# eduardburlacu/DiTSep

Hardware: AMD Instinct MI355X
Metric: separated utterances/sec @ N=30, 2-spk 4 s mixtures (higher is better)
Workload: dtype fp16 (fp16 MFMA operands, fp32 accumulate)

## Files before the change

ditsep_amd/csrc/common.h:

```cpp
#pragma once
#include <hip/hip_runtime.h>
#include <stdint.h>

typedef unsigned short op16_t;
typedef __attribute__((ext_vector_type(8))) unsigned short op16x8;
typedef __attribute__((ext_vector_type(4))) unsigned short op16x4;
typedef __attribute__((ext_vector_type(8))) __bf16 bf16x8;
typedef __attribute__((ext_vector_type(8))) _Float16 f16x8;
typedef __attribute__((ext_vector_type(4))) float f32x4;

#define DSN_WAVE 64

#define DSN_PL(planes, f16) ((planes) | ((f16) << 4))
#define PL_COUNT(pl) ((pl)&3)
#define PL_F16(pl) ((pl) >> 4)

enum { DSN_ACT_NONE = 0, DSN_ACT_ELU = 1, DSN_ACT_SNAKE = 2, DSN_ACT_SILU = 3 };
enum { DSN_F32_NONE = 0, DSN_F32_TANH = 1 };

__device__ __forceinline__ float dsn_elu(float v) { return v > 0.f ? v : expm1f(v); }
__device__ __forceinline__ float dsn_silu(float v) { return v / (1.f + __expf(-v)); }
__device__ __forceinline__ float dsn_snake(float v, float alpha, float inv_beta) {
  float s = __sinf(v * alpha);
  return v + inv_beta * s * s;
}

#define DSN_F16_MAX 65504.f
__device__ __forceinline__ float dsn_sat16(float v) {
  const float c = __builtin_amdgcn_fmed3f(v, -DSN_F16_MAX, DSN_F16_MAX);
  return v != v ? v : c;
}
__device__ __forceinline__ op16_t to_op16(float v, int f16) {
  return f16 ? __builtin_bit_cast(unsigned short, (_Float16)dsn_sat16(v)) : __builtin_bit_cast(unsigned short, (__bf16)v);
}
__device__ __forceinline__ float from_op16(op16_t u, int f16) {
// ... 167 lines not shown
```

ditsep_amd/csrc/engine.hip:

```cpp
#include <math.h>
#include <stdarg.h>
#include <stdio.h>
#include <stdlib.h>
#include <string.h>

#include <algorithm>
#include <map>
#include <numeric>
#include <set>
#include <stdexcept>
#include <string>
#include <vector>

#include "../../include/ditsep_hip.h"
#include "dit_plan.h"
#include "igemm.h"
#include "kernels.h"
#include "resample_plan.h"
#include "score_window.h"

namespace {

struct Err : std::runtime_error {
  int code;
// ... 4241 lines not shown
                 (int)h[i], (long)h[i] * t->mul, t->L);
        const char* why = launch_codec_tail_zero(oplanes, t->out_ps, P, t->x, t->out_f32, t->B, t->L, t->C,
                                                 reinterpret_cast<const int*>(t->lens), t->rep, t->mul, st);
        if (why) fail(DSN_EINVAL, "test_kernel codec_tail_zero: %s (C=%d)", why, t->C);
        break;
      }
      case DSN_TK_RANDN:
      case DSN_TK_RAND_UNIFORM: {
        const char* nm = t->kind == DSN_TK_RANDN ? "randn" : "rand_uniform";
        if (t->count < 1) fail(DSN_EINVAL, "test_kernel %s: count %ld must be positive", nm, (long)t->count);
        if (!t->out_f32) fail(DSN_EINVAL, "test_kernel %s: out_f32 missing", nm);
        if (t->kind == DSN_TK_RANDN) launch_randn(t->out_f32, (long)t->count, t->seed, t->offset, st);
        else launch_rand_uniform(t->out_f32, (long)t->count, t->seed, t->offset, t->lo, t->hi, st);
        break;
      }
      case DSN_TK_WN_SCALE: {
        if (t->rows < 1 || t->count < 1)
          fail(DSN_EINVAL, "test_kernel wn_scale: rows and count must be positive (rows=%d count=%ld)", t->rows, (long)t->count);
        if (!t->x || !t->gamma || !t->out_f32) fail(DSN_EINVAL, "test_kernel wn_scale: x (v), gamma (g) or out_f32 missing");
        launch_wn_scale(t->x, t->gamma, t->out_f32, t->rows, (long)t->count, st);
        break;
      }
      case DSN_TK_PACK_WEIGHT: {
        static const char* const modes[] = {"linear", "linear_swiglu", "conv", "convt", "conv2d", "nin"};
        const int m = t->mode, N = t->N, K = t->K;
        if (m < PACK_LINEAR || m > PACK_NIN) fail(DSN_EINVAL, "test_kernel pack_weight: unknown mode %d", m);
        if (N < 1 || K < 1) fail(DSN_EINVAL, "test_kernel pack_weight %s: N and K must be positive (N=%d K=%d)", modes[m], N, K);
        if (!t->x || !oplanes) fail(DSN_EINVAL, "test_kernel pack_weight %s: x (the source) or out_planes missing", modes[m]);
        if (t->out_ps < (long)N * K) fail(DSN_EINVAL, "test_kernel pack_weight %s: out_ps %ld < N*K", modes[m], (long)t->out_ps);
        const bool linear = m == PACK_LINEAR || m == PACK_LINEAR_SWIGLU;
// ... 279 lines not shown
```

ditsep_amd/csrc/kernels.h:

```cpp
#pragma once
#include "common.h"

void launch_pack_tokens(const float* src0, int C0, const float* src1, int C1, int B, int T,
                        float* dst_f32, op16_t* dst_planes, long ps, int planes, hipStream_t s);
void launch_win_pack_tokens(const float* src0, int C0, const float* src1, int C1, const int* wtab, int W, int Tw,
                            int Tsrc, float* dst_f32, op16_t* dst_planes, long ps, int planes, hipStream_t s);
void launch_win_times(const float* t, const int* wtab, int W, float* tw, hipStream_t s);
void launch_win_blend_tokens(const float* src, const int* ftab, const float* fw, float* out, long rows, int C, int Tw,
                             hipStream_t s);
void launch_copy_rows(const float* src, float* dst, int rows, int width, long dst_stride, hipStream_t s);
void launch_unpack_tokens(const float* src, float* dst, int B, int C, int T, hipStream_t s);
void launch_to_planes(const float* src, op16_t* dst, long ps, int planes, long n, hipStream_t s);

void launch_pc_prior(const float* mean, int mean_full, const float* z, float* x, float stdT, int B, int n, int D,
                     int T, hipStream_t s);
void launch_pc_corrector(float* x, float* x_mean , const float* score_tok, const float* z, float step,
                         float noise_gain, const float* norms, float snr, int B, int n, int D, int T, hipStream_t s);
void launch_pc_item_norms(const float* a, long per_item, int B, float* out, hipStream_t s);
void launch_pc_predictor(float* x, float* x_mean, const float* y, const float* score_tok, const float* z,
                         float theta, float dt, float G, float g, int em, int B, int n, int D, int T, hipStream_t s);

void launch_sigma_mix(const float* y, float* smix, int B, int L, int avg_len, hipStream_t s);
void launch_mix_prior(const float* y, const float* z, float* x, const float* smix, float s1, float s2, int B, int n, int D,
                      int T, hipStream_t s);
// ... 10 lines not shown
void launch_residual_norm(float* x, const float* slabs, int nslab, long slab_stride, const float* bias,
                          const float* gamma, const float* beta, op16_t* out, long ps, int planes, int rows, int D,
                          float eps, int do_norm, hipStream_t s, unsigned char* out_fp8_scale = nullptr);
void launch_timestep_features(const float* t, const float* w, int B, int half, op16_t* out, long ps,
                              int planes, hipStream_t s);
hipError_t launch_attention_mfma(const op16_t* qkv, long ps, op16_t* out, long out_ps, int pl, int B, int S, int H,
                                 int dh, hipStream_t s, unsigned char* out_fp8_scale = nullptr,
                                 const int* lens = nullptr);
void launch_rope_tables(float* cos_t, float* sin_t, int S, int rot, hipStream_t s);

void launch_conv_out1(const op16_t* a, long ps, int planes, const float* w, float* out, int S, int L, int C,
                      int ktaps, int apply_tanh, hipStream_t s);
void launch_conv_in1(const float* wav, const float* w, const float* bias, int S, int L, int Cout, int ktaps,
                     float* out_f32, op16_t* out_planes, long ps, int planes, int act, const float* act_a,
                     const float* act_b, hipStream_t s);
void launch_vae_sample(const float* enc_tok, const float* noise, float* y, int S, int D, int T, hipStream_t s);

const char* launch_codec_tail_zero(op16_t* planes, long ps, int n_planes, float* xf, float* out, int S, int L, int C,
                                   const int* frames, int rep, int mul, hipStream_t s);
void launch_vae_sample_ragged(const float* enc_tok, const float* noise, const int* frames, float* y, int S, int D, int T,
                              hipStream_t s);

void launch_randn(float* out, long n, unsigned long long seed, unsigned long long offset, hipStream_t s);

enum { PACK_LINEAR = 0, PACK_LINEAR_SWIGLU = 1, PACK_CONV = 2, PACK_CONVT = 3, PACK_CONV2D = 4, PACK_NIN = 5 };
void launch_wn_scale(const float* v, const float* g, float* scale, int R, long inner, hipStream_t s);
void launch_pack_weight(const float* src, const float* scale, op16_t* dst, long ps, int planes, int mode,
                        int N, int K, int Cin, int Cout, int kw, int stride, hipStream_t s,
                        const float* colscale = nullptr);
void launch_packed_row_sum(const op16_t* w, long ps, int planes, int N, int K, float* out, hipStream_t s);
// ... 246 lines not shown
```

ditsep_amd/csrc/kernels.hip:

```cpp
#include "kernels.h"

namespace {

constexpr int TPB = 256;
inline int grid_for(long n, int per_block = TPB, int cap = 256 * 16) {
  long g = (n + per_block - 1) / per_block;
  return (int)(g < 1 ? 1 : (g > cap ? cap : g));
}


template <bool WIN>
__global__ void pack_tokens_kernel(const float* __restrict__ s0, int C0, const float* __restrict__ s1, int C1,
                                   int B, int T, float* __restrict__ df, op16_t* __restrict__ dp, long ps,
                                   int planes, const int* __restrict__ wtab, int Tsrc) {
  const int C = C0 + C1;
  const long n = (long)B * T * C;
  for (long i = blockIdx.x * (long)blockDim.x + threadIdx.x; i < n; i += (long)gridDim.x * blockDim.x) {
    const int c = (int)(i % C);
    const long bt = i / C;
    const int t = (int)(bt % T);
    const int b = (int)(bt / T);
    float v;
    if (WIN) {
      const int r = wtab[3 * b], ts = wtab[3 * b + 1] + t;
// ... 606 lines not shown
      if (q == 0) part[r * 8 + t] = x;
    }
  }
  __syncthreads();
  for (int p = threadIdx.x; p < TILE; p += blockDim.x) {
    const int l = l0 + p;
    if (l < L) {
      float v = 0.f;
#pragma unroll
      for (int t = 0; t < KT; ++t) v += part[(p + t) * 8 + t];
      out[(long)s * L + l] = apply_tanh ? tanhf(v) : v;
    }
  }
}

__global__ void conv_in1_kernel(const float* __restrict__ wav, const float* __restrict__ w,
                                const float* __restrict__ bias, int L, int Cout, int ktaps,
                                float* __restrict__ of, op16_t* __restrict__ op, long ps, int planes, int act,
                                const float* __restrict__ aa, const float* __restrict__ ab, long total) {
  const int pad = (ktaps - 1) / 2;
  for (long i = blockIdx.x * (long)blockDim.x + threadIdx.x; i < total; i += (long)gridDim.x * blockDim.x) {
    const int co = (int)(i % Cout);
    const long sl = i / Cout;
    const int l = (int)(sl % L);
    const long s = sl / L;
    float acc = bias ? bias[co] : 0.f;
    for (int t = 0; t < ktaps; ++t) {
      const int li = l + t - pad;
      if (li >= 0 && li < L) acc += w[co * ktaps + t] * wav[s * L + li];
    }
    if (of) of[i] = acc;
    if (op) {
      float a = acc;
      if (act == DSN_ACT_ELU) a = dsn_elu(acc);
      else if (act == DSN_ACT_SNAKE) a = dsn_snake(acc, aa[co], ab[co]);
      dsn_store_planes1(op, ps, planes, i, a);
    }
  }
}

__global__ void conv_in1_vec_kernel(const float* __restrict__ wav, const float* __restrict__ w,
                                    const float* __restrict__ bias, int L, int Cout, int ktaps,
                                    float* __restrict__ of, op16_t* __restrict__ op, long ps, int planes, int act,
                                    const float* __restrict__ aa, const float* __restrict__ ab, long rows) {
  const int cq = Cout >> 2;
  const int c4 = (threadIdx.x % cq) * 4;
  const int pad = (ktaps - 1) / 2;
  float wr[4][8];
  f32x4 bv = {0.f, 0.f, 0.f, 0.f};
#pragma unroll
  for (int r = 0; r < 4; ++r) {
#pragma unroll
    for (int t = 0; t < 8; ++t) wr[r][t] = t < ktaps ? w[(c4 + r) * ktaps + t] : 0.f;
    if (bias) bv[r] = bias[c4 + r];
  }
  const int rpb = blockDim.x / cq;
  for (long row = blockIdx.x * (long)rpb + threadIdx.x / cq; row < rows; row += (long)gridDim.x * rpb) {
    const int l = (int)(row % L);
    const long s = row / L;
// ... 3 lines not shown
      const int li = l + t - pad;
      x[t] = (t < ktaps && li >= 0 && li < L) ? wav[s * L + li] : 0.f;
    }
    f32x4 acc = bv;
#pragma unroll
    for (int r = 0; r < 4; ++r)
#pragma unroll
      for (int t = 0; t < 8; ++t) acc[r] += wr[r][t] * x[t];
    const long o = row * Cout + c4;
    if (of) *reinterpret_cast<f32x4*>(of + o) = acc;
    if (op) {
      op16x4 hi, lo;
#pragma unroll
      for (int r = 0; r < 4; ++r) {
        float v = acc[r];
        if (act == DSN_ACT_ELU) v = dsn_elu(v);
        else if (act == DSN_ACT_SNAKE) v = dsn_snake(v, aa[c4 + r], ab[c4 + r]);
        op16_t h, lw;
        dsn_split(v, h, lw, PL_F16(planes));
        hi[r] = h;
        lo[r] = lw;
      }
      *reinterpret_cast<op16x4*>(op + o) = hi;
      if (PL_COUNT(planes) == 2) *reinterpret_cast<op16x4*>(op + ps + o) = lo;
    }
  }
}

__global__ void vae_sample_kernel(const float* __restrict__ enc, const float* __restrict__ noise,
                                  float* __restrict__ y, int D, int T, long total) {
  for (long i = blockIdx.x * (long)blockDim.x + threadIdx.x; i < total; i += (long)gridDim.x * blockDim.x) {
    const int t = (int)(i % T);
    const long sc = i / T;
    const int c = (int)(sc % D);
    const long s = sc / D;
    const float* row = enc + (s * T + t) * (2L * D);
    const float mean = row[c], scale = row[D + c];
    const float sp = scale > 20.f ? scale : log1pf(expf(scale));
    y[i] = noise[i] * (sp + 1e-4f) + mean;
  }
// ... 342 lines not shown
                     apply_tanh);
}
void launch_conv_in1(const float* wav, const float* w, const float* bias, int S, int L, int Cout, int ktaps,
                     float* of, op16_t* op, long ps, int planes, int act, const float* aa, const float* ab,
                     hipStream_t st) {
  if (Cout % 4 == 0 && TPB % (Cout / 4) == 0 && ktaps <= 8) {
    const long rows = (long)S * L;
    hipLaunchKernelGGL(conv_in1_vec_kernel, dim3(grid_for(rows * (Cout / 4))), dim3(TPB), 0, st, wav, w, bias, L, Cout,
                       ktaps, of, op, ps, planes, act, aa, ab, rows);
    return;
  }
  const long total = (long)S * L * Cout;
  hipLaunchKernelGGL(conv_in1_kernel, dim3(grid_for(total)), dim3(TPB), 0, st, wav, w, bias, L, Cout, ktaps, of, op,
                     ps, planes, act, aa, ab, total);
}
void launch_vae_sample(const float* enc, const float* noise, float* y, int S, int D, int T, hipStream_t st) {
  const long total = (long)S * D * T;
  hipLaunchKernelGGL(vae_sample_kernel, dim3(grid_for(total)), dim3(TPB), 0, st, enc, noise, y, D, T, total);
}
void launch_randn(float* out, long n, unsigned long long seed, unsigned long long offset, hipStream_t st) {
  hipLaunchKernelGGL(randn_kernel, dim3(grid_for((n + 3) / 4)), dim3(TPB), 0, st, out, n, seed, offset);
}
void launch_rand_uniform(float* out, long n, unsigned long long seed, unsigned long long offset, float lo, float hi,
                         hipStream_t st) {
  hipLaunchKernelGGL(rand_uniform_kernel, dim3(grid_for(n)), dim3(TPB), 0, st, out, n, seed, offset, lo, hi);
}
void launch_wn_scale(const float* v, const float* g, float* scale, int R, long inner, hipStream_t st) {
  hipLaunchKernelGGL(wn_scale_kernel, dim3(cdiv(R, 4)), dim3(TPB), 0, st, v, g, scale, R, inner);
}
void launch_pack_weight(const float* src, const float* scale, op16_t* dst, long ps, int planes, int mode, int N,
// ... 71 lines not shown
```

ditsep_amd/csrc/ru_fused.hip:

```cpp
#include "igemm.h"
#include "kernels.h"
#include <cstdlib>
#include <functional>

namespace {

constexpr int C = 128;
constexpr int TL = 128;
constexpr int KT = 32;
constexpr int WTILE = 128 * KT;
constexpr int NSTW = 3;

__device__ __forceinline__ int swz32(int row, int chunk) { return chunk ^ ((-(row >> 2)) & 3); }

template <int P, int F16>
__global__ __launch_bounds__(256, 2) void ru_fused_kernel(const RuDesc d, const op16_t* __restrict__ zero_page) {
  extern __shared__ __attribute__((aligned(16))) op16_t lds[];
  const int halo = 3 * d.dil;
  const int hrows = (TL + 2 * halo + 3) & ~3;
  constexpr int AH_ROWS = TL + 54 + 2;
  constexpr int AH_PLANE = AH_ROWS * C;
  op16_t* ah = lds;
  op16_t* ring = lds + P * AH_PLANE;
  constexpr int RING_STAGE = P * WTILE;

  const int tid = threadIdx.x, lane = tid & 63;
  const int wave = __builtin_amdgcn_readfirstlane(tid >> 6);
  const int wm = wave >> 1, wn = wave & 1;
  const int tiles_per_seq = (d.L + TL - 1) / TL;
  const int s = blockIdx.x / tiles_per_seq;
// ... 73 lines not shown
#pragma unroll
      for (int tm = 0; tm < 4; ++tm) {
        if (P == 2) {
          acc[tn][tm] = mfma16<F16>(fw[P - 1][tn], fa[0][tm], acc[tn][tm]);
          acc[tn][tm] = mfma16<F16>(fw[0][tn], fa[P - 1][tm], acc[tn][tm]);
        }
        acc[tn][tm] = mfma16<F16>(fw[0][tn], fa[0][tm], acc[tn][tm]);
      }
  }
  asm volatile("s_waitcnt lgkmcnt(0)" ::: "memory");
  __builtin_amdgcn_s_barrier();

  issue_w(d.W1, d.w1_ps, C, 0, 0);
  issue_w(d.W1, d.w1_ps, C, KT, 1);
  const int nq = (lane >> 4) * 4;
#pragma unroll
  for (int tm = 0; tm < 4; ++tm) {
    const int m = wm * 64 + tm * 16 + (lane & 15);
#pragma unroll
    for (int tn = 0; tn < 4; ++tn) {
      const int n = wn * 64 + tn * 16 + nq;
      f32x4 v = acc[tn][tm] + *reinterpret_cast<const f32x4*>(d.b7 + n);
      op16x4 hi, lo;
#pragma unroll
      for (int r = 0; r < 4; ++r) {
        float a = v[r];
        if (d.act_mid == DSN_ACT_ELU) a = dsn_elu(a);
        else if (d.act_mid == DSN_ACT_SNAKE) a = dsn_snake(a, d.mid_a[n + r], d.mid_b[n + r]);
        op16_t h, l;
        dsn_split(a, h, l, F16);
        hi[r] = h;
        lo[r] = l;
      }
      const int off = m * C + (((n >> 3) + 2 * m) & 15) * 8 + (n & 7);
      *reinterpret_cast<op16x4*>(ah + off) = hi;
      if (P == 2) *reinterpret_cast<op16x4*>(ah + AH_PLANE + off) = lo;
      acc[tn][tm] = f32x4{0.f, 0.f, 0.f, 0.f};
    }
  }

  constexpr int NKT1 = C / KT;
  for (int i = 0; i < NKT1; ++i) {
    if (i + 1 < NKT1)
      asm volatile("s_waitcnt vmcnt(%0) lgkmcnt(0)" ::"n"(G) : "memory");
    else
      asm volatile("s_waitcnt vmcnt(0) lgkmcnt(0)" ::: "memory");
    __builtin_amdgcn_s_barrier();
    if (i + 2 < NKT1) issue_w(d.W1, d.w1_ps, C, (i + 2) * KT, (i + 2) % NSTW);
// ... 7 lines not shown
        fa[p][k] = *reinterpret_cast<const op16x8*>(ah + p * AH_PLANE + row * C + ((i * 4 + fchunk + 2 * row) & 15) * 8);
        fw[p][k] = *reinterpret_cast<const op16x8*>(wb + p * WTILE + w_frag + k * 16 * KT);
      }
#pragma unroll
    for (int tn = 0; tn < 4; ++tn)
#pragma unroll
      for (int tm = 0; tm < 4; ++tm) {
        if (P == 2) {
          acc[tn][tm] = mfma16<F16>(fw[P - 1][tn], fa[0][tm], acc[tn][tm]);
          acc[tn][tm] = mfma16<F16>(fw[0][tn], fa[P - 1][tm], acc[tn][tm]);
        }
        acc[tn][tm] = mfma16<F16>(fw[0][tn], fa[0][tm], acc[tn][tm]);
      }
  }

  f32x4 res[4], nres[4];
  auto load_res = [&](int tm, f32x4 (&r)[4]) {
    const int l = l0 + wm * 64 + tm * 16 + (lane & 15);
    const long rowoff = seq_off + (long)min(l, d.L - 1) * C;
#pragma unroll
    for (int tn = 0; tn < 4; ++tn) r[tn] = *reinterpret_cast<const f32x4*>(d.X + rowoff + wn * 64 + tn * 16 + nq);
  };
  load_res(0, res);
#pragma unroll
  for (int tm = 0; tm < 4; ++tm) {
    if (tm + 1 < 4) load_res(tm + 1, nres);
    const int l = l0 + wm * 64 + tm * 16 + (lane & 15);
    const long rowoff = seq_off + (long)l * C;
#pragma unroll
    for (int tn = 0; tn < 4; ++tn) {
      if (l >= d.L) continue;
      const int n = wn * 64 + tn * 16 + nq;
      f32x4 v = acc[tn][tm] + *reinterpret_cast<const f32x4*>(d.b1 + n) + res[tn];
      if (d.out_f32) *reinterpret_cast<f32x4*>(d.out_f32 + rowoff + n) = v;
      if (d.out_planes) {
        op16x4 hi, lo;
#pragma unroll
        for (int r = 0; r < 4; ++r) {
          float a = v[r];
          if (d.act_out == DSN_ACT_ELU) a = dsn_elu(a);
          else if (d.act_out == DSN_ACT_SNAKE) a = dsn_snake(a, d.out_a[n + r], d.out_b[n + r]);
          op16_t h, lw;
          dsn_split(a, h, lw, F16);
          hi[r] = h;
          lo[r] = lw;
        }
        *reinterpret_cast<op16x4*>(d.out_planes + rowoff + n) = hi;
        if (P == 2) *reinterpret_cast<op16x4*>(d.out_planes + d.out_ps + rowoff + n) = lo;
      }
    }
#pragma unroll
    for (int tn = 0; tn < 4; ++tn) res[tn] = nres[tn];
  }
}

constexpr int TL2 = 256;
constexpr int ACH_ROWS = 384;
constexpr int ACH_STAGE = ACH_ROWS * KT;
constexpr int RING2_OFF = 2 * ACH_STAGE;
constexpr int H_ELEMS = TL2 * C;
constexpr int LDS2_ELEMS = H_ELEMS + 2 * WTILE;

template <int F16>
__global__ __launch_bounds__(512, 4) void ru_fused2_kernel(const RuDesc d, const op16_t* __restrict__ zero_page) {
  extern __shared__ __attribute__((aligned(16))) op16_t lds[];
  const int halo = 3 * d.dil;
  const int tid = threadIdx.x, lane = tid & 63;
  const int wave = __builtin_amdgcn_readfirstlane(tid >> 6);
  const int wm = wave >> 1, wn = wave & 1;
  const int tiles_per_seq = (d.L + TL2 - 1) / TL2;
  const int s = blockIdx.x / tiles_per_seq;
  const int l0 = (blockIdx.x - s * tiles_per_seq) * TL2;
  const long seq_off = (long)s * d.L * C;
  const int nrows = TL2 + 2 * halo;

  const op16_t* a_src[3];
#pragma unroll
  for (int j = 0; j < 3; ++j) {
// ... 63 lines not shown
      }
#pragma unroll
      for (int tn = 0; tn < 4; ++tn)
#pragma unroll
        for (int tm = 0; tm < 4; ++tm) acc[tn][tm] = mfma16<F16>(fw[tn], fa[tm], acc[tn][tm]);
      if (++st == NSTW) st = 0;
    }
  }
  asm volatile("s_waitcnt lgkmcnt(0)" ::: "memory");
  __builtin_amdgcn_s_barrier();

  op16_t* ring1 = lds + H_ELEMS;
  issue_w(d.W1, C, 0, ring1);
  issue_w(d.W1, C, KT, ring1 + WTILE);
  const int nq = (lane >> 4) * 4;
#pragma unroll
  for (int tm = 0; tm < 4; ++tm) {
    const int m = wm * 64 + tm * 16 + (lane & 15);
#pragma unroll
    for (int tn = 0; tn < 4; ++tn) {
      const int n = wn * 64 + tn * 16 + nq;
      f32x4 v = acc[tn][tm] + *reinterpret_cast<const f32x4*>(d.b7 + n);
      op16x4 hi;
#pragma unroll
      for (int r = 0; r < 4; ++r) {
        float a = v[r];
        if (d.act_mid == DSN_ACT_ELU) a = dsn_elu(a);
        else if (d.act_mid == DSN_ACT_SNAKE) a = dsn_snake(a, d.mid_a[n + r], d.mid_b[n + r]);
        op16_t h, l;
        dsn_split(a, h, l, F16);
        hi[r] = h;
      }
      *reinterpret_cast<op16x4*>(lds + m * C + (((n >> 3) + 2 * m) & 15) * 8 + (n & 7)) = hi;
      const int ls = l0 + wm * 64 + tm * 16 + (lane & 15);
      acc[tn][tm] = *reinterpret_cast<const f32x4*>(d.b1 + n) +
                    *reinterpret_cast<const f32x4*>(d.X + seq_off + (long)min(ls, d.L - 1) * C + n);
    }
  }

#pragma unroll
  for (int i = 0; i < 4; ++i) {
    if (i == 0)
      asm volatile("s_waitcnt vmcnt(1) lgkmcnt(0)" ::: "memory");
    else
      asm volatile("s_waitcnt vmcnt(0) lgkmcnt(0)" ::: "memory");
    __builtin_amdgcn_s_barrier();
    if (i >= 1 && i + 1 < 4) issue_w(d.W1, C, (i + 1) * KT, ring1 + ((i + 1) & 1) * WTILE);
    const op16_t* wb = ring1 + (i & 1) * WTILE;
    op16x8 fa[4], fw[4];
#pragma unroll
    for (int k = 0; k < 4; ++k) {
      const int row = wm * 64 + k * 16 + frow;
      fa[k] = *reinterpret_cast<const op16x8*>(lds + row * C + ((i * 4 + fchunk + 2 * row) & 15) * 8);
      fw[k] = *reinterpret_cast<const op16x8*>(wb + w_frag + k * 16 * KT);
    }
#pragma unroll
    for (int tn = 0; tn < 4; ++tn)
#pragma unroll
      for (int tm = 0; tm < 4; ++tm) acc[tn][tm] = mfma16<F16>(fw[tn], fa[tm], acc[tn][tm]);
  }

#pragma unroll
  for (int tm = 0; tm < 4; ++tm) {
    const int l = l0 + wm * 64 + tm * 16 + (lane & 15);
    const long rowoff = seq_off + (long)l * C;
#pragma unroll
    for (int tn = 0; tn < 4; ++tn) {
      if (l >= d.L) continue;
      const int n = wn * 64 + tn * 16 + nq;
      const f32x4 v = acc[tn][tm];
      if (d.out_f32) *reinterpret_cast<f32x4*>(d.out_f32 + rowoff + n) = v;
      if (d.out_planes) {
        op16x4 hi;
#pragma unroll
        for (int r = 0; r < 4; ++r) {
          float a = v[r];
          if (d.act_out == DSN_ACT_ELU) a = dsn_elu(a);
          else if (d.act_out == DSN_ACT_SNAKE) a = dsn_snake(a, d.out_a[n + r], d.out_b[n + r]);
          op16_t h, lw;
          dsn_split(a, h, lw, F16);
          hi[r] = h;
        }
        *reinterpret_cast<op16x4*>(d.out_planes + rowoff + n) = hi;
      }
    }
  }
}

template <int P, int F16>
hipError_t launch_t(const RuDesc& d, hipStream_t st) {
  const op16_t* zp = dsn_zero_page();
  if (!zp) return hipErrorOutOfMemory;
  const size_t smem = ((size_t)P * (TL + 56) * C + (size_t)NSTW * P * WTILE) * sizeof(op16_t);
  dsn_allow_lds<ru_fused_kernel<P, F16>>();
  const int grid = d.S * ((d.L + TL - 1) / TL);
  hipLaunchKernelGGL((ru_fused_kernel<P, F16>), dim3(grid), dim3(256), smem, st, d, zp);
  return hipGetLastError();
}

}

template <int F16>
hipError_t launch2_t(const RuDesc& d, hipStream_t st) {
  const op16_t* zp = dsn_zero_page();
  if (!zp) return hipErrorOutOfMemory;
  const size_t smem = (size_t)LDS2_ELEMS * sizeof(op16_t);
  dsn_allow_lds<ru_fused2_kernel<F16>>();
  const int grid = d.S * ((d.L + TL2 - 1) / TL2);
  hipLaunchKernelGGL((ru_fused2_kernel<F16>), dim3(grid), dim3(512), smem, st, d, zp);
  return hipGetLastError();
}

static bool ru_act_ok(int kind, const float* a, const float* b) {
  if (kind == DSN_ACT_SNAKE) return a && b;
  return kind == DSN_ACT_NONE || kind == DSN_ACT_ELU;
}

hipError_t ru_fused_launch(const RuDesc& d, int pl, bool v1, hipStream_t st) {
  if (d.dil < 1 || d.dil > 9 || d.S <= 0 || d.L <= 0) return hipErrorInvalidValue;
  if (!d.A || !d.X || !d.W7 || !d.W1 || !d.b7 || !d.b1 || (!d.out_f32 && !d.out_planes)) return hipErrorInvalidValue;
  if (!ru_act_ok(d.act_mid, d.mid_a, d.mid_b)) return hipErrorInvalidValue;
  if (d.out_planes && !ru_act_ok(d.act_out, d.out_a, d.out_b)) return hipErrorInvalidValue;
  const int P = PL_COUNT(pl), f16 = PL_F16(pl);
  if (d.out_planes) {
    const long n = (long)d.S * d.L * C;
    for (int p = 0; p < P; ++p)
      for (int q = 0; q < P; ++q) {
        const op16_t *a = d.A + p * d.a_ps, *o = d.out_planes + q * d.out_ps;
        if (std::less<const op16_t*>()(a, o + n) && std::less<const op16_t*>()(o, a + n)) return hipErrorInvalidValue;
      }
  }
  if (P == 1 && !v1) return f16 ? launch2_t<1>(d, st) : launch2_t<0>(d, st);
  if (P == 1) return f16 ? launch_t<1, 1>(d, st) : launch_t<1, 0>(d, st);
  return f16 ? launch_t<2, 1>(d, st) : launch_t<2, 0>(d, st);
}
```

ditsep_amd/native.py:

```python
from __future__ import annotations

import ctypes as C
import math
import os
import warnings
from typing import Mapping, Optional

import torch

_HERE = os.path.dirname(os.path.abspath(__file__))
LIB_PATH = os.environ.get("DSN_LIB", os.path.join(_HERE, "libditsep_hip.so"))

PREC_BF16 = 1
PREC_BF16X3 = 2
PREC_FP16 = 3
PREC_FP16X3 = 4
PREC_FP8 = 5
SCORE_NONE, SCORE_DIT, SCORE_NCSNPP = 0, 1, 2
MAX_VAE_BLOCKS = 8

EXPORTS = [
    "dsn_create", "dsn_destroy", "dsn_last_error", "dsn_load_tensor", "dsn_finalize_weights", "dsn_finalize_weights_ex",
    "dsn_score", "dsn_score_ragged", "dsn_pc_sample_ragged", "dsn_decode_ragged", "dsn_encode_ragged",
    "dsn_separate_ragged", "dsn_ouve_schedule", "dsn_pc_sample", "dsn_pc_sample_sched", "dsn_pc_sample_ex", "dsn_pc_sample_mix", "dsn_sb_sample", "dsn_decode",
# ... 134 lines not shown
        ("sc_Cin", C.c_int), ("sc_row_elems", C.c_int),
        ("out_f32", C.c_void_p), ("out_planes", C.c_void_p), ("out_ps", C.c_int64),
        ("slabs", C.c_void_p), ("slab_stride", C.c_int64),
    ]


TEST_KERNEL_KINDS = {"attention": 1, "qkv_attention": 2, "residual_norm": 3, "gn_stats": 4, "gn_apply": 5, "fir2d": 6,
                     "conv_out1": 7, "conv_in1": 8, "ru_fused": 9,
                     "pc_prior": 10, "pc_corrector": 11, "pc_item_norms": 12, "pc_predictor": 13, "sigma_mix": 14,
                     "mix_prior": 15, "mix_corrector": 16, "mix_predictor": 17, "sb_update": 18, "repeat_sources": 19,
                     "vae_sample": 20, "randn": 21, "rand_uniform": 22, "codec_tail_zero": 23,
                     "wn_scale": 24, "pack_weight": 25, "pack_bias_swiglu": 26, "pack_weight_fp8": 27,
                     "packed_row_sum": 28, "fp8_row_sum": 29, "bias_plus_wbeta": 30, "snake_params": 31,
                     "pack_tokens": 32, "unpack_tokens": 33, "copy_rows": 34, "to_planes": 35, "zero_tail": 36,
                     "vae_sample_ragged": 37, "timestep_features": 38, "rope_tables": 39, "ncsn_pack": 40,
                     "ncsn_fourier": 41, "ncsn_output": 42, "win_pack_tokens": 43, "win_blend_tokens": 44}
PACK_MODES = {"linear": 0, "linear_swiglu": 1, "conv": 2, "convt": 3, "conv2d": 4, "nin": 5}


class DsnTestKernel(C.Structure):
    _fields_ = [
        ("kind", C.c_int), ("B", C.c_int), ("S", C.c_int), ("H", C.c_int), ("dh", C.c_int), ("D", C.c_int),
        ("ipp", C.c_int), ("rows", C.c_int), ("nslab", C.c_int), ("do_norm", C.c_int), ("eps", C.c_float),
        ("slab_stride", C.c_int64),
        ("C", C.c_int), ("HW", C.c_int), ("rstride", C.c_int), ("img_h", C.c_int), ("img_w", C.c_int), ("up", C.c_int),
        ("silu", C.c_int), ("bstride", C.c_int64),
        ("L", C.c_int), ("ktaps", C.c_int), ("apply_tanh", C.c_int), ("act", C.c_int),
        ("dil", C.c_int), ("act_out", C.c_int),
        ("a", C.c_void_p), ("a_numel", C.c_int64), ("w", C.c_void_p), ("w_numel", C.c_int64), ("w2", C.c_void_p),
        ("w2_numel", C.c_int64), ("x", C.c_void_p),
        ("slabs", C.c_void_p), ("bias", C.c_void_p), ("bias2", C.c_void_p), ("gamma", C.c_void_p), ("beta", C.c_void_p),
# ... 1880 lines not shown
```

include/ditsep_hip.h:

```cpp
#ifndef DITSEP_HIP_H
#define DITSEP_HIP_H

#include <stdint.h>

#ifdef __cplusplus
extern "C" {
#endif

#define DSN_OK 0
#define DSN_EINVAL (-1)
#define DSN_EHIP (-2)
#define DSN_ESTATE (-3)
#define DSN_ENOMEM (-4)
#define DSN_ESOLVER (-5)

#define DSN_PREC_BF16 1
#define DSN_PREC_BF16X3 2
#define DSN_PREC_FP16 3
#define DSN_PREC_FP16X3 4
#define DSN_PREC_FP8 5

#define DSN_SCORE_NONE 0
#define DSN_SCORE_DIT 1
#define DSN_SCORE_NCSNPP 2
// ... 302 lines not shown
  int64_t slab_stride;
} DsnTestGemm;
int dsn_test_gemm(dsn_ctx* ctx, const DsnTestGemm* t, void* stream);

enum { DSN_TK_ATTENTION = 1, DSN_TK_QKV_ATTENTION = 2, DSN_TK_RESIDUAL_NORM = 3, DSN_TK_GN_STATS = 4,
       DSN_TK_GN_APPLY = 5, DSN_TK_FIR2D = 6, DSN_TK_CONV_OUT1 = 7, DSN_TK_CONV_IN1 = 8, DSN_TK_RU_FUSED = 9,
       DSN_TK_PC_PRIOR = 10, DSN_TK_PC_CORRECTOR = 11, DSN_TK_PC_ITEM_NORMS = 12, DSN_TK_PC_PREDICTOR = 13,
       DSN_TK_SIGMA_MIX = 14, DSN_TK_MIX_PRIOR = 15, DSN_TK_MIX_CORRECTOR = 16, DSN_TK_MIX_PREDICTOR = 17,
       DSN_TK_SB_UPDATE = 18, DSN_TK_REPEAT_SOURCES = 19, DSN_TK_VAE_SAMPLE = 20, DSN_TK_RANDN = 21,
       DSN_TK_RAND_UNIFORM = 22, DSN_TK_CODEC_TAIL_ZERO = 23,
       DSN_TK_WN_SCALE = 24, DSN_TK_PACK_WEIGHT = 25, DSN_TK_PACK_BIAS_SWIGLU = 26, DSN_TK_PACK_WEIGHT_FP8 = 27,
       DSN_TK_PACKED_ROW_SUM = 28, DSN_TK_FP8_ROW_SUM = 29, DSN_TK_BIAS_PLUS_WBETA = 30, DSN_TK_SNAKE_PARAMS = 31,
       DSN_TK_PACK_TOKENS = 32, DSN_TK_UNPACK_TOKENS = 33, DSN_TK_COPY_ROWS = 34, DSN_TK_TO_PLANES = 35,
       DSN_TK_ZERO_TAIL = 36, DSN_TK_VAE_SAMPLE_RAGGED = 37, DSN_TK_TIMESTEP_FEATURES = 38, DSN_TK_ROPE_TABLES = 39,
       DSN_TK_NCSN_PACK = 40, DSN_TK_NCSN_FOURIER = 41, DSN_TK_NCSN_OUTPUT = 42, DSN_TK_WIN_PACK_TOKENS = 43,
       DSN_TK_WIN_BLEND_TOKENS = 44 };
enum { DSN_PACK_LINEAR = 0, DSN_PACK_LINEAR_SWIGLU = 1, DSN_PACK_CONV = 2, DSN_PACK_CONVT = 3, DSN_PACK_CONV2D = 4,
       DSN_PACK_NIN = 5 };
typedef struct DsnTestKernel {
  int kind;
  int B, S, H, dh, D, ipp;
  int rows, nslab, do_norm;
  float eps;
  int64_t slab_stride;
  int C, HW, rstride, img_h, img_w, up, silu;
  int64_t bstride;
  int L, ktaps, apply_tanh, act;
  int dil, act_out;
  const float* a;
  int64_t a_numel;
  const float* w;
// ... 74 lines not shown
```

Before: 290.6.

## Specialize residual-unit epilogues by activation mode and inline a branch-free ELU expm1

Replaces the library expm1f in ELU with an inlined Cody-Waite plus polynomial expm1 for non-positive inputs, adding a sweep kernel that compares it bit-for-bit against the reference. The fused residual-unit kernels and the conv_in1 kernels are templated on activation mode, so the activation and output-pointer branches resolve at compile time. Snake alpha/beta are loaded once as vectors instead of per element. This cuts per-element branching and scalar parameter loads in the epilogues, at the cost of more kernel instantiations and code size.

```diff
diff --git a/ditsep_amd/csrc/common.h b/ditsep_amd/csrc/common.h
--- a/ditsep_amd/csrc/common.h
+++ b/ditsep_amd/csrc/common.h
@@ -18,7 +18,28 @@
 enum { DSN_ACT_NONE = 0, DSN_ACT_ELU = 1, DSN_ACT_SNAKE = 2, DSN_ACT_SILU = 3 };
 enum { DSN_F32_NONE = 0, DSN_F32_TANH = 1 };
 
-__device__ __forceinline__ float dsn_elu(float v) { return v > 0.f ? v : expm1f(v); }
+__device__ __forceinline__ float dsn_expm1_nonpos(float x) {
+  const auto c = [](unsigned bits) { return __builtin_bit_cast(float, bits); };
+  const float t = __builtin_rintf(x * c(0x3fb8aa3bu));
+  float r = __builtin_fmaf(t, c(0xbf317218u), x);
+  r = __builtin_fmaf(t, c(0x3102e308u), r);
+  float p = __builtin_fmaf(c(0x395133b1u), r, c(0x3ab69700u));
+  p = __builtin_fmaf(r, p, c(0x3c0887f9u));
+  p = __builtin_fmaf(r, p, c(0x3d2aaa81u));
+  p = __builtin_fmaf(r, p, c(0x3e2aaaabu));
+  p = __builtin_fmaf(r, p, 0.5f);
+  const float q = r * p;
+  const float u = __builtin_fmaf(r, q, r);
+  const float s = __builtin_amdgcn_ldexpf(1.0f, (int)t);
+  const float y = __builtin_fmaf(s, u, s - 1.0f);
+  return x < -17.0f ? -1.0f : y;
+}
+__device__ __forceinline__ float dsn_elu(float v) {
+  float e = dsn_expm1_nonpos(v > 0.f ? 0.f : v);
+  asm("" : "+v"(e));
+  return v > 0.f ? v : e;
+}
+__device__ __forceinline__ float dsn_elu_ref(float v) { return v > 0.f ? v : expm1f(v); }
 __device__ __forceinline__ float dsn_silu(float v) { return v / (1.f + __expf(-v)); }
 __device__ __forceinline__ float dsn_snake(float v, float alpha, float inv_beta) {
   float s = __sinf(v * alpha);
diff --git a/ditsep_amd/csrc/engine.hip b/ditsep_amd/csrc/engine.hip
--- a/ditsep_amd/csrc/engine.hip
+++ b/ditsep_amd/csrc/engine.hip
@@ -4279,6 +4279,15 @@
         else launch_rand_uniform(t->out_f32, (long)t->count, t->seed, t->offset, t->lo, t->hi, st);
         break;
       }
+      case DSN_TK_ELU_SWEEP: {
+        if (t->count < 1 || t->count > (1ll << 32) || t->offset + (uint64_t)t->count > (1ull << 32))
+          fail(DSN_EINVAL, "test_kernel elu_sweep: patterns offset .. offset + count - 1 must lie in [0, 2^32) (count=%ld)",
+               (long)t->count);
+        if (!t->out_f32 || (reinterpret_cast<uintptr_t>(t->out_f32) & 7))
+          fail(DSN_EINVAL, "test_kernel elu_sweep: out_f32 (16 bytes, 8-byte aligned) missing");
+        launch_elu_sweep(t->offset, (unsigned long long)t->count, reinterpret_cast<unsigned long long*>(t->out_f32), st);
+        break;
+      }
       case DSN_TK_WN_SCALE: {
         if (t->rows < 1 || t->count < 1)
           fail(DSN_EINVAL, "test_kernel wn_scale: rows and count must be positive (rows=%d count=%ld)", t->rows, (long)t->count);
diff --git a/ditsep_amd/csrc/kernels.h b/ditsep_amd/csrc/kernels.h
--- a/ditsep_amd/csrc/kernels.h
+++ b/ditsep_amd/csrc/kernels.h
@@ -48,6 +48,7 @@
 void launch_conv_in1(const float* wav, const float* w, const float* bias, int S, int L, int Cout, int ktaps,
                      float* out_f32, op16_t* out_planes, long ps, int planes, int act, const float* act_a,
                      const float* act_b, hipStream_t s);
+void launch_elu_sweep(unsigned long long first, unsigned long long count, unsigned long long* res, hipStream_t s);
 void launch_vae_sample(const float* enc_tok, const float* noise, float* y, int S, int D, int T, hipStream_t s);
 
 const char* launch_codec_tail_zero(op16_t* planes, long ps, int n_planes, float* xf, float* out, int S, int L, int C,
diff --git a/ditsep_amd/csrc/kernels.hip b/ditsep_amd/csrc/kernels.hip
--- a/ditsep_amd/csrc/kernels.hip
+++ b/ditsep_amd/csrc/kernels.hip
@@ -644,10 +644,11 @@
   }
 }
 
-__global__ void conv_in1_kernel(const float* __restrict__ wav, const float* __restrict__ w,
-                                const float* __restrict__ bias, int L, int Cout, int ktaps,
-                                float* __restrict__ of, op16_t* __restrict__ op, long ps, int planes, int act,
-                                const float* __restrict__ aa, const float* __restrict__ ab, long total) {
+template <int ACT>
+__device__ __forceinline__ void conv_in1_loop(const float* __restrict__ wav, const float* __restrict__ w,
+                                              const float* __restrict__ bias, int L, int Cout, int ktaps,
+                                              float* __restrict__ of, op16_t* __restrict__ op, long ps, int planes,
+                                              const float* __restrict__ aa, const float* __restrict__ ab, long total) {
   const int pad = (ktaps - 1) / 2;
   for (long i = blockIdx.x * (long)blockDim.x + threadIdx.x; i < total; i += (long)gridDim.x * blockDim.x) {
     const int co = (int)(i % Cout);
@@ -662,17 +663,26 @@
     if (of) of[i] = acc;
     if (op) {
       float a = acc;
-      if (act == DSN_ACT_ELU) a = dsn_elu(acc);
-      else if (act == DSN_ACT_SNAKE) a = dsn_snake(acc, aa[co], ab[co]);
+      if (ACT == DSN_ACT_ELU) a = dsn_elu(acc);
+      else if (ACT == DSN_ACT_SNAKE) a = dsn_snake(acc, aa[co], ab[co]);
       dsn_store_planes1(op, ps, planes, i, a);
     }
   }
 }
-
-__global__ void conv_in1_vec_kernel(const float* __restrict__ wav, const float* __restrict__ w,
-                                    const float* __restrict__ bias, int L, int Cout, int ktaps,
-                                    float* __restrict__ of, op16_t* __restrict__ op, long ps, int planes, int act,
-                                    const float* __restrict__ aa, const float* __restrict__ ab, long rows) {
+__global__ void conv_in1_kernel(const float* __restrict__ wav, const float* __restrict__ w,
+                                const float* __restrict__ bias, int L, int Cout, int ktaps,
+                                float* __restrict__ of, op16_t* __restrict__ op, long ps, int planes, int act,
+                                const float* __restrict__ aa, const float* __restrict__ ab, long total) {
+  if (act == DSN_ACT_ELU) conv_in1_loop<DSN_ACT_ELU>(wav, w, bias, L, Cout, ktaps, of, op, ps, planes, aa, ab, total);
+  else if (act == DSN_ACT_SNAKE) conv_in1_loop<DSN_ACT_SNAKE>(wav, w, bias, L, Cout, ktaps, of, op, ps, planes, aa, ab, total);
+  else conv_in1_loop<DSN_ACT_NONE>(wav, w, bias, L, Cout, ktaps, of, op, ps, planes, aa, ab, total);
+}
+
+template <int ACT>
+__device__ __forceinline__ void conv_in1_vec_loop(const float* __restrict__ wav, const float* __restrict__ w,
+                                                  const float* __restrict__ bias, int L, int Cout, int ktaps,
+                                                  float* __restrict__ of, op16_t* __restrict__ op, long ps, int planes,
+                                                  const float* __restrict__ aa, const float* __restrict__ ab, long rows) {
   const int cq = Cout >> 2;
   const int c4 = (threadIdx.x % cq) * 4;
   const int pad = (ktaps - 1) / 2;
@@ -706,8 +716,8 @@
 #pragma unroll
       for (int r = 0; r < 4; ++r) {
         float v = acc[r];
-        if (act == DSN_ACT_ELU) v = dsn_elu(v);
-        else if (act == DSN_ACT_SNAKE) v = dsn_snake(v, aa[c4 + r], ab[c4 + r]);
+        if (ACT == DSN_ACT_ELU) v = dsn_elu(v);
+        else if (ACT == DSN_ACT_SNAKE) v = dsn_snake(v, aa[c4 + r], ab[c4 + r]);
         op16_t h, lw;
         dsn_split(v, h, lw, PL_F16(planes));
         hi[r] = h;
@@ -716,6 +726,33 @@
       *reinterpret_cast<op16x4*>(op + o) = hi;
       if (PL_COUNT(planes) == 2) *reinterpret_cast<op16x4*>(op + ps + o) = lo;
     }
+  }
+}
+__global__ void conv_in1_vec_kernel(const float* __restrict__ wav, const float* __restrict__ w,
+                                    const float* __restrict__ bias, int L, int Cout, int ktaps,
+                                    float* __restrict__ of, op16_t* __restrict__ op, long ps, int planes, int act,
+                                    const float* __restrict__ aa, const float* __restrict__ ab, long rows) {
+  if (act == DSN_ACT_ELU) conv_in1_vec_loop<DSN_ACT_ELU>(wav, w, bias, L, Cout, ktaps, of, op, ps, planes, aa, ab, rows);
+  else if (act == DSN_ACT_SNAKE) conv_in1_vec_loop<DSN_ACT_SNAKE>(wav, w, bias, L, Cout, ktaps, of, op, ps, planes, aa, ab, rows);
+  else conv_in1_vec_loop<DSN_ACT_NONE>(wav, w, bias, L, Cout, ktaps, of, op, ps, planes, aa, ab, rows);
+}
+
+__global__ void elu_sweep_kernel(unsigned long long first, unsigned long long count, unsigned long long* __restrict__ res) {
+  unsigned long long bad = 0, lowest = ~0ull;
+  for (unsigned long long i = blockIdx.x * (unsigned long long)blockDim.x + threadIdx.x; i < count;
+       i += (unsigned long long)gridDim.x * blockDim.x) {
+    const unsigned pat = (unsigned)(first + i);
+    const float v = __builtin_bit_cast(float, pat);
+    const float got = dsn_elu(v), want = dsn_elu_ref(v);
+    const bool same = __builtin_bit_cast(unsigned, got) == __builtin_bit_cast(unsigned, want) || (got != got && want != want);
+    if (!same) {
+      ++bad;
+      lowest = pat < lowest ? pat : lowest;
+    }
+  }
+  if (bad) {
+    atomicAdd(res, bad);
+    atomicMin(res + 1, lowest);
   }
 }
 
@@ -1088,6 +1125,11 @@
   hipLaunchKernelGGL(conv_in1_kernel, dim3(grid_for(total)), dim3(TPB), 0, st, wav, w, bias, L, Cout, ktaps, of, op,
                      ps, planes, act, aa, ab, total);
 }
+void launch_elu_sweep(unsigned long long first, unsigned long long count, unsigned long long* res, hipStream_t st) {
+  (void)hipMemsetAsync(res, 0, sizeof *res, st);
+  (void)hipMemsetAsync(res + 1, 0xff, sizeof *res, st);
+  hipLaunchKernelGGL(elu_sweep_kernel, dim3(grid_for((long)((count + 15) / 16))), dim3(TPB), 0, st, first, count, res);
+}
 void launch_vae_sample(const float* enc, const float* noise, float* y, int S, int D, int T, hipStream_t st) {
   const long total = (long)S * D * T;
   hipLaunchKernelGGL(vae_sample_kernel, dim3(grid_for(total)), dim3(TPB), 0, st, enc, noise, y, D, T, total);
diff --git a/ditsep_amd/csrc/ru_fused.hip b/ditsep_amd/csrc/ru_fused.hip
--- a/ditsep_amd/csrc/ru_fused.hip
+++ b/ditsep_amd/csrc/ru_fused.hip
@@ -13,7 +13,57 @@
 
 __device__ __forceinline__ int swz32(int row, int chunk) { return chunk ^ ((-(row >> 2)) & 3); }
 
-template <int P, int F16>
+enum { RU_ANY = 0, RU_ELU_BOTH = 1, RU_ELU_PLANES = 2, RU_SNAKE_BOTH = 3, RU_SNAKE_PLANES = 4 };
+template <int MODE>
+__device__ __forceinline__ int ru_kind(int runtime_kind) {
+  return MODE == RU_ANY ? runtime_kind : (MODE == RU_ELU_BOTH || MODE == RU_ELU_PLANES) ? DSN_ACT_ELU : DSN_ACT_SNAKE;
+}
+template <int MODE>
+__device__ __forceinline__ bool ru_writes_f32(const RuDesc& d) {
+  return MODE == RU_ANY ? d.out_f32 != nullptr : (MODE == RU_ELU_BOTH || MODE == RU_SNAKE_BOTH);
+}
+template <int MODE>
+__device__ __forceinline__ bool ru_writes_planes(const RuDesc& d) {
+  return MODE == RU_ANY ? d.out_planes != nullptr : true;
+}
+__device__ __forceinline__ void ru_snake_vecs(bool snake, const float* a, const float* b, f32x4 (&sa)[4], f32x4 (&sb)[4]) {
+#pragma unroll
+  for (int tn = 0; tn < 4; ++tn) {
+    sa[tn] = sb[tn] = f32x4{0.f, 0.f, 0.f, 0.f};
+    if (snake) {
+      sa[tn] = *reinterpret_cast<const f32x4*>(a + tn * 16);
+      sb[tn] = *reinterpret_cast<const f32x4*>(b + tn * 16);
+    }
+  }
+}
+__device__ __forceinline__ f32x4 ru_act4(int kind, const f32x4& v, const f32x4& alpha, const f32x4& inv_beta) {
+  f32x4 a = v;
+  if (kind == DSN_ACT_ELU) {
+#pragma unroll
+    for (int r = 0; r < 4; ++r) a[r] = dsn_elu(v[r]);
+  } else if (kind == DSN_ACT_SNAKE) {
+#pragma unroll
+    for (int r = 0; r < 4; ++r) a[r] = dsn_snake(v[r], alpha[r], inv_beta[r]);
+  }
+  return a;
+}
+__device__ __forceinline__ f32x4 ru_add4(const f32x4& a, const f32x4& b) {
+  f32x4 c;
+#pragma unroll
+  for (int r = 0; r < 4; ++r) c[r] = a[r] + b[r];
+  return c;
+}
+__device__ __forceinline__ void ru_split4(const f32x4& a, op16x4& hi, op16x4& lo, int f16) {
+#pragma unroll
+  for (int r = 0; r < 4; ++r) {
+    op16_t h, l;
+    dsn_split(a[r], h, l, f16);
+    hi[r] = h;
+    lo[r] = l;
+  }
+}
+
+template <int P, int F16, int MODE>
 __global__ __launch_bounds__(256, 2) void ru_fused_kernel(const RuDesc d, const op16_t* __restrict__ zero_page) {
   extern __shared__ __attribute__((aligned(16))) op16_t lds[];
   const int halo = 3 * d.dil;
@@ -117,24 +167,19 @@
   issue_w(d.W1, d.w1_ps, C, 0, 0);
   issue_w(d.W1, d.w1_ps, C, KT, 1);
   const int nq = (lane >> 4) * 4;
+  const int cb = wn * 64 + nq;
+  f32x4 sa[4], sb[4];
+  const int kmid = ru_kind<MODE>(d.act_mid);
+  ru_snake_vecs(kmid == DSN_ACT_SNAKE, d.mid_a + cb, d.mid_b + cb, sa, sb);
 #pragma unroll
   for (int tm = 0; tm < 4; ++tm) {
     const int m = wm * 64 + tm * 16 + (lane & 15);
 #pragma unroll
     for (int tn = 0; tn < 4; ++tn) {
-      const int n = wn * 64 + tn * 16 + nq;
-      f32x4 v = acc[tn][tm] + *reinterpret_cast<const f32x4*>(d.b7 + n);
+      const int n = cb + tn * 16;
+      const f32x4 v = ru_add4(acc[tn][tm], *reinterpret_cast<const f32x4*>(d.b7 + n));
       op16x4 hi, lo;
-#pragma unroll
-      for (int r = 0; r < 4; ++r) {
-        float a = v[r];
-        if (d.act_mid == DSN_ACT_ELU) a = dsn_elu(a);
-        else if (d.act_mid == DSN_ACT_SNAKE) a = dsn_snake(a, d.mid_a[n + r], d.mid_b[n + r]);
-        op16_t h, l;
-        dsn_split(a, h, l, F16);
-        hi[r] = h;
-        lo[r] = l;
-      }
+      ru_split4(ru_act4(kmid, v, sa[tn], sb[tn]), hi, lo, F16);
       const int off = m * C + (((n >> 3) + 2 * m) & 15) * 8 + (n & 7);
       *reinterpret_cast<op16x4*>(ah + off) = hi;
       if (P == 2) *reinterpret_cast<op16x4*>(ah + AH_PLANE + off) = lo;
@@ -172,39 +217,33 @@
       }
   }
 
+  const bool wf = ru_writes_f32<MODE>(d), wp = ru_writes_planes<MODE>(d);
+  const int kout = ru_kind<MODE>(d.act_out);
+  ru_snake_vecs(wp && kout == DSN_ACT_SNAKE, d.out_a + cb, d.out_b + cb, sa, sb);
   f32x4 res[4], nres[4];
   auto load_res = [&](int tm, f32x4 (&r)[4]) {
     const int l = l0 + wm * 64 + tm * 16 + (lane & 15);
-    const long rowoff = seq_off + (long)min(l, d.L - 1) * C;
-#pragma unroll
-    for (int tn = 0; tn < 4; ++tn) r[tn] = *reinterpret_cast<const f32x4*>(d.X + rowoff + wn * 64 + tn * 16 + nq);
+    const float* xrow = d.X + seq_off + (long)min(l, d.L - 1) * C + cb;
+#pragma unroll
+    for (int tn = 0; tn < 4; ++tn) r[tn] = *reinterpret_cast<const f32x4*>(xrow + tn * 16);
   };
   load_res(0, res);
 #pragma unroll
   for (int tm = 0; tm < 4; ++tm) {
     if (tm + 1 < 4) load_res(tm + 1, nres);
     const int l = l0 + wm * 64 + tm * 16 + (lane & 15);
-    const long rowoff = seq_off + (long)l * C;
-#pragma unroll
-    for (int tn = 0; tn < 4; ++tn) {
-      if (l >= d.L) continue;
-      const int n = wn * 64 + tn * 16 + nq;
-      f32x4 v = acc[tn][tm] + *reinterpret_cast<const f32x4*>(d.b1 + n) + res[tn];
-      if (d.out_f32) *reinterpret_cast<f32x4*>(d.out_f32 + rowoff + n) = v;
-      if (d.out_planes) {
-        op16x4 hi, lo;
-#pragma unroll
-        for (int r = 0; r < 4; ++r) {
-          float a = v[r];
-          if (d.act_out == DSN_ACT_ELU) a = dsn_elu(a);
-          else if (d.act_out == DSN_ACT_SNAKE) a = dsn_snake(a, d.out_a[n + r], d.out_b[n + r]);
-          op16_t h, lw;
-          dsn_split(a, h, lw, F16);
-          hi[r] = h;
-          lo[r] = lw;
+    const long rowoff = seq_off + (long)l * C + cb;
+    if (l < d.L) {
+#pragma unroll
+      for (int tn = 0; tn < 4; ++tn) {
+        const f32x4 v = ru_add4(ru_add4(acc[tn][tm], *reinterpret_cast<const f32x4*>(d.b1 + cb + tn * 16)), res[tn]);
+        if (wf) *reinterpret_cast<f32x4*>(d.out_f32 + rowoff + tn * 16) = v;
+        if (wp) {
+          op16x4 hi, lo;
+          ru_split4(ru_act4(kout, v, sa[tn], sb[tn]), hi, lo, F16);
+          *reinterpret_cast<op16x4*>(d.out_planes + rowoff + tn * 16) = hi;
+          if (P == 2) *reinterpret_cast<op16x4*>(d.out_planes + d.out_ps + rowoff + tn * 16) = lo;
         }
-        *reinterpret_cast<op16x4*>(d.out_planes + rowoff + n) = hi;
-        if (P == 2) *reinterpret_cast<op16x4*>(d.out_planes + d.out_ps + rowoff + n) = lo;
       }
     }
 #pragma unroll
@@ -219,7 +258,7 @@
 constexpr int H_ELEMS = TL2 * C;
 constexpr int LDS2_ELEMS = H_ELEMS + 2 * WTILE;
 
-template <int F16>
+template <int F16, int MODE>
 __global__ __launch_bounds__(512, 4) void ru_fused2_kernel(const RuDesc d, const op16_t* __restrict__ zero_page) {
   extern __shared__ __attribute__((aligned(16))) op16_t lds[];
   const int halo = 3 * d.dil;
@@ -313,27 +352,22 @@
   issue_w(d.W1, C, 0, ring1);
   issue_w(d.W1, C, KT, ring1 + WTILE);
   const int nq = (lane >> 4) * 4;
+  const int cb = wn * 64 + nq;
+  f32x4 sa[4], sb[4];
+  const int kmid = ru_kind<MODE>(d.act_mid);
+  ru_snake_vecs(kmid == DSN_ACT_SNAKE, d.mid_a + cb, d.mid_b + cb, sa, sb);
 #pragma unroll
   for (int tm = 0; tm < 4; ++tm) {
     const int m = wm * 64 + tm * 16 + (lane & 15);
+    const float* xrow = d.X + seq_off + (long)min(l0 + m, d.L - 1) * C + cb;
 #pragma unroll
     for (int tn = 0; tn < 4; ++tn) {
-      const int n = wn * 64 + tn * 16 + nq;
-      f32x4 v = acc[tn][tm] + *reinterpret_cast<const f32x4*>(d.b7 + n);
-      op16x4 hi;
-#pragma unroll
-      for (int r = 0; r < 4; ++r) {
-        float a = v[r];
-        if (d.act_mid == DSN_ACT_ELU) a = dsn_elu(a);
-        else if (d.act_mid == DSN_ACT_SNAKE) a = dsn_snake(a, d.mid_a[n + r], d.mid_b[n + r]);
-        op16_t h, l;
-        dsn_split(a, h, l, F16);
-        hi[r] = h;
-      }
+      const int n = cb + tn * 16;
+      const f32x4 v = ru_add4(acc[tn][tm], *reinterpret_cast<const f32x4*>(d.b7 + n));
+      op16x4 hi, lo;
+      ru_split4(ru_act4(kmid, v, sa[tn], sb[tn]), hi, lo, F16);
       *reinterpret_cast<op16x4*>(lds + m * C + (((n >> 3) + 2 * m) & 15) * 8 + (n & 7)) = hi;
-      const int ls = l0 + wm * 64 + tm * 16 + (lane & 15);
-      acc[tn][tm] = *reinterpret_cast<const f32x4*>(d.b1 + n) +
-                    *reinterpret_cast<const f32x4*>(d.X + seq_off + (long)min(ls, d.L - 1) * C + n);
+      acc[tn][tm] = ru_add4(*reinterpret_cast<const f32x4*>(d.b1 + n), *reinterpret_cast<const f32x4*>(xrow + tn * 16));
     }
   }
 
@@ -359,55 +393,73 @@
       for (int tm = 0; tm < 4; ++tm) acc[tn][tm] = mfma16<F16>(fw[tn], fa[tm], acc[tn][tm]);
   }
 
+  const bool wf = ru_writes_f32<MODE>(d), wp = ru_writes_planes<MODE>(d);
+  const int kout = ru_kind<MODE>(d.act_out);
+  ru_snake_vecs(wp && kout == DSN_ACT_SNAKE, d.out_a + cb, d.out_b + cb, sa, sb);
 #pragma unroll
   for (int tm = 0; tm < 4; ++tm) {
     const int l = l0 + wm * 64 + tm * 16 + (lane & 15);
-    const long rowoff = seq_off + (long)l * C;
+    if (l >= d.L) continue;
+    const long rowoff = seq_off + (long)l * C + cb;
+    float* const orow = d.out_f32 + rowoff;
+    op16_t* const prow = d.out_planes + rowoff;
 #pragma unroll
     for (int tn = 0; tn < 4; ++tn) {
-      if (l >= d.L) continue;
-      const int n = wn * 64 + tn * 16 + nq;
       const f32x4 v = acc[tn][tm];
-      if (d.out_f32) *reinterpret_cast<f32x4*>(d.out_f32 + rowoff + n) = v;
-      if (d.out_planes) {
-        op16x4 hi;
-#pragma unroll
-        for (int r = 0; r < 4; ++r) {
-          float a = v[r];
-          if (d.act_out == DSN_ACT_ELU) a = dsn_elu(a);
-          else if (d.act_out == DSN_ACT_SNAKE) a = dsn_snake(a, d.out_a[n + r], d.out_b[n + r]);
-          op16_t h, lw;
-          dsn_split(a, h, lw, F16);
-          hi[r] = h;
-        }
-        *reinterpret_cast<op16x4*>(d.out_planes + rowoff + n) = hi;
-      }
-    }
-  }
-}
-
-template <int P, int F16>
+      if (wf) *reinterpret_cast<f32x4*>(orow + tn * 16) = v;
+      if (wp) {
+        op16x4 hi, lo;
+        ru_split4(ru_act4(kout, v, sa[tn], sb[tn]), hi, lo, F16);
+        *reinterpret_cast<op16x4*>(prow + tn * 16) = hi;
+      }
+    }
+  }
+}
+
+template <int P, int F16, int MODE>
 hipError_t launch_t(const RuDesc& d, hipStream_t st) {
   const op16_t* zp = dsn_zero_page();
   if (!zp) return hipErrorOutOfMemory;
   const size_t smem = ((size_t)P * (TL + 56) * C + (size_t)NSTW * P * WTILE) * sizeof(op16_t);
-  dsn_allow_lds<ru_fused_kernel<P, F16>>();
+  dsn_allow_lds<ru_fused_kernel<P, F16, MODE>>();
   const int grid = d.S * ((d.L + TL - 1) / TL);
-  hipLaunchKernelGGL((ru_fused_kernel<P, F16>), dim3(grid), dim3(256), smem, st, d, zp);
+  hipLaunchKernelGGL((ru_fused_kernel<P, F16, MODE>), dim3(grid), dim3(256), smem, st, d, zp);
   return hipGetLastError();
 }
 
-}
-
-template <int F16>
+template <int F16, int MODE>
 hipError_t launch2_t(const RuDesc& d, hipStream_t st) {
   const op16_t* zp = dsn_zero_page();
   if (!zp) return hipErrorOutOfMemory;
   const size_t smem = (size_t)LDS2_ELEMS * sizeof(op16_t);
-  dsn_allow_lds<ru_fused2_kernel<F16>>();
+  dsn_allow_lds<ru_fused2_kernel<F16, MODE>>();
   const int grid = d.S * ((d.L + TL2 - 1) / TL2);
-  hipLaunchKernelGGL((ru_fused2_kernel<F16>), dim3(grid), dim3(512), smem, st, d, zp);
+  hipLaunchKernelGGL((ru_fused2_kernel<F16, MODE>), dim3(grid), dim3(512), smem, st, d, zp);
   return hipGetLastError();
+}
+
+int ru_mode(const RuDesc& d) {
+  if (!d.out_planes || d.act_mid != d.act_out) return RU_ANY;
+  if (d.act_mid == DSN_ACT_ELU) return d.out_f32 ? RU_ELU_BOTH : RU_ELU_PLANES;
+  if (d.act_mid == DSN_ACT_SNAKE) return d.out_f32 ? RU_SNAKE_BOTH : RU_SNAKE_PLANES;
+  return RU_ANY;
+}
+template <int P, int F16, int MODE>
+hipError_t launch_one(const RuDesc& d, hipStream_t st) {
+  if constexpr (P == 0) return launch2_t<F16, MODE>(d, st);
+  else return launch_t<P, F16, MODE>(d, st);
+}
+template <int P, int F16>
+hipError_t launch_mode(const RuDesc& d, hipStream_t st) {
+  switch (ru_mode(d)) {
+    case RU_ELU_BOTH: return launch_one<P, F16, RU_ELU_BOTH>(d, st);
+    case RU_ELU_PLANES: return launch_one<P, F16, RU_ELU_PLANES>(d, st);
+    case RU_SNAKE_BOTH: return launch_one<P, F16, RU_SNAKE_BOTH>(d, st);
+    case RU_SNAKE_PLANES: return launch_one<P, F16, RU_SNAKE_PLANES>(d, st);
+    default: return launch_one<P, F16, RU_ANY>(d, st);
+  }
+}
+
 }
 
 static bool ru_act_ok(int kind, const float* a, const float* b) {
@@ -429,7 +481,7 @@
         if (std::less<const op16_t*>()(a, o + n) && std::less<const op16_t*>()(o, a + n)) return hipErrorInvalidValue;
       }
   }
-  if (P == 1 && !v1) return f16 ? launch2_t<1>(d, st) : launch2_t<0>(d, st);
-  if (P == 1) return f16 ? launch_t<1, 1>(d, st) : launch_t<1, 0>(d, st);
-  return f16 ? launch_t<2, 1>(d, st) : launch_t<2, 0>(d, st);
-}
+  if (P == 1 && !v1) return f16 ? launch_mode<0, 1>(d, st) : launch_mode<0, 0>(d, st);
+  if (P == 1) return f16 ? launch_mode<1, 1>(d, st) : launch_mode<1, 0>(d, st);
+  return f16 ? launch_mode<2, 1>(d, st) : launch_mode<2, 0>(d, st);
+}
diff --git a/ditsep_amd/native.py b/ditsep_amd/native.py
--- a/ditsep_amd/native.py
+++ b/ditsep_amd/native.py
@@ -172,7 +172,7 @@
                      "packed_row_sum": 28, "fp8_row_sum": 29, "bias_plus_wbeta": 30, "snake_params": 31,
                      "pack_tokens": 32, "unpack_tokens": 33, "copy_rows": 34, "to_planes": 35, "zero_tail": 36,
                      "vae_sample_ragged": 37, "timestep_features": 38, "rope_tables": 39, "ncsn_pack": 40,
-                     "ncsn_fourier": 41, "ncsn_output": 42, "win_pack_tokens": 43, "win_blend_tokens": 44}
+                     "ncsn_fourier": 41, "ncsn_output": 42, "win_pack_tokens": 43, "win_blend_tokens": 44, "elu_sweep": 45}
 PACK_MODES = {"linear": 0, "linear_swiglu": 1, "conv": 2, "convt": 3, "conv2d": 4, "nin": 5}
 
 
diff --git a/include/ditsep_hip.h b/include/ditsep_hip.h
--- a/include/ditsep_hip.h
+++ b/include/ditsep_hip.h
@@ -340,7 +340,7 @@
        DSN_TK_PACK_TOKENS = 32, DSN_TK_UNPACK_TOKENS = 33, DSN_TK_COPY_ROWS = 34, DSN_TK_TO_PLANES = 35,
        DSN_TK_ZERO_TAIL = 36, DSN_TK_VAE_SAMPLE_RAGGED = 37, DSN_TK_TIMESTEP_FEATURES = 38, DSN_TK_ROPE_TABLES = 39,
        DSN_TK_NCSN_PACK = 40, DSN_TK_NCSN_FOURIER = 41, DSN_TK_NCSN_OUTPUT = 42, DSN_TK_WIN_PACK_TOKENS = 43,
-       DSN_TK_WIN_BLEND_TOKENS = 44 };
+       DSN_TK_WIN_BLEND_TOKENS = 44, DSN_TK_ELU_SWEEP = 45 };
 enum { DSN_PACK_LINEAR = 0, DSN_PACK_LINEAR_SWIGLU = 1, DSN_PACK_CONV = 2, DSN_PACK_CONVT = 3, DSN_PACK_CONV2D = 4,
        DSN_PACK_NIN = 5 };
 typedef struct DsnTestKernel {
```

Result: no change. 287.8 (-1.0%).
